# dan11003/tbv_slam_public

Measured on AMD Instinct MI355X. Metric: radar scan registrations/sec (400x3360 polar), higher is better.
Workload: dtype u8 filter / f32 search / f64 solve

## Files before the change

### tbv_slam_public_amd/csrc/kstrong.hip

```cpp
#include <cmath>

#include "polar_common.hpp"

namespace {

struct KStrongArgs {
  const uint8_t* polar;
  int rows, cols, stride, batch;
  long long batch_stride;
  int k, u_zmin, want_peaks, batch0;
  int32_t* sel_range;
  uint8_t* sel_intensity;
  int32_t* sel_count;
  uint8_t* is_peak;
  int32_t* row_valid;
  int min_range_bin;
  int dense_halo;
  uint32_t* row_keys;
  const long long* image_offsets;
};

__device__ __forceinline__ uint32_t swar_ge(uint32_t x, uint32_t tl4, bool thi) {
  const uint32_t g = ((x & 0x7f7f7f7fu) | 0x80808080u) - tl4;
  const uint32_t xh = x & 0x80808080u;
// ... 78 lines not shown
  const bool do_peaks = !STAGED && a.want_peaks && a.is_peak;
  uint8_t halo = 0;
  int halo_pos = 0;
  if (do_peaks && (lane < 6 || (lane >= 8 && lane < 14))) {
    const long long total = (long long)a.rows * a.stride;
    long long lin;
    if (lane < 6) {
      halo_pos = -6 + lane;
      lin = row_lin - 6 + lane;
      if (a.dense_halo) lin = r > 0 ? row_lin - a.stride + a.cols - 6 + lane : -1;
    } else {
      halo_pos = a.cols + (lane - 8);
      lin = row_lin + halo_pos;
      if (a.dense_halo) lin = r + 1 < a.rows ? row_lin + a.stride + (lane - 8) : total;
    }
    if (lin >= 0 && lin < total) halo = img[lin];
  }
  const int cols16 = (a.cols + 15) & ~15;
  uint32_t w[NCHUNK * 4];
  if (STAGED) {
#pragma unroll
    for (int c = 0; c < NCHUNK; c++) {
      uint4 v = make_uint4(0, 0, 0, 0);
      if ((c * 64 + lane) * 16 < cols16) v = *(const uint4*)(rowbuf + (c * 64 + lane) * 16);
      w[c * 4] = v.x; w[c * 4 + 1] = v.y; w[c * 4 + 2] = v.z; w[c * 4 + 3] = v.w;
    }
  } else {
    load_row<NCHUNK, VEC>(rowp, a.cols, lane, w, cfear_piece_inside_image(r, a.cols & ~15, a.rows, a.stride));
#pragma unroll
    for (int c = 0; c < NCHUNK; c++)
      *(uint4*)(rowbuf + (c * 64 + lane) * 16) = make_uint4(w[c * 4], w[c * 4 + 1], w[c * 4 + 2], w[c * 4 + 3]);
  }

  auto reload_row = [&](uint32_t (&x)[NCHUNK * 4]) {
#pragma unroll
    for (int c = 0; c < NCHUNK; c++) {
      uint4 v = make_uint4(0, 0, 0, 0);
      if (!STAGED || (c * 64 + lane) * 16 < cols16) v = *(const uint4*)(rowbuf + (c * 64 + lane) * 16);
      x[c * 4] = v.x; x[c * 4 + 1] = v.y; x[c * 4 + 2] = v.z; x[c * 4 + 3] = v.w;
    }
  };
  uint32_t bm[NCHUNK];
  {
    const uint32_t tz4 = (uint32_t)(a.u_zmin & 0x7f) * 0x01010101u;
    if (a.u_zmin & 0x80) candidate_bitmaps<NCHUNK, MASK, true>(w, tz4, a.cols, lane, bm);
    else candidate_bitmaps<NCHUNK, MASK, false>(w, tz4, a.cols, lane, bm);
  }
  int c_lane = 0;
#pragma unroll
  for (int c = 0; c < NCHUNK; c++) c_lane += __popc(bm[c]);
  const int c_incl = wave_incl_scan_i32(c_lane);
  const int n_ge = __builtin_amdgcn_readlane(c_incl, 63);
  int n_sel;
  int n_all;
  __builtin_amdgcn_fence(__ATOMIC_RELEASE, "wavefront");
  __builtin_amdgcn_wave_barrier();
  __builtin_amdgcn_fence(__ATOMIC_ACQUIRE, "wavefront");

  uint8_t* marker = (uint8_t*)hist;
  uint32_t* sexcl = hist + 64;
  uint32_t* spw = hist + 128;
  auto scatter_prepare = [&](const uint32_t (&bmx)[NCHUNK], int cnt_lane, int cnt_incl) {
    uint32_t pw[NP];
#pragma unroll
    for (int p = 0; p < NP; p++) pw[p] = (bmx[2 * p] >> 4) | (2 * p + 1 < NCHUNK ? bmx[2 * p + 1] : 0u);
    const int excl = cnt_incl - cnt_lane;
    ((uint32_t*)marker)[lane] = 0;
// ... 47 lines not shown
    const int s_incl = wave_incl_scan_i32(s_lane);
    const unsigned long long reach = __ballot(s_incl >= k);
    const int lc = __ffsll((long long)reach) - 1;
    int Tl = 0, gl = 0, el = 0;
    {
      int cum = s_incl - s_lane;
      const int hv[4] = {(int)h.w, (int)h.z, (int)h.y, (int)h.x};
      bool found = false;
#pragma unroll
      for (int j = 0; j < 4; j++) {
        if (!found && cum + hv[j] >= k) { Tl = 4 * (63 - lane) + 3 - j; gl = cum; el = hv[j]; found = true; }
        cum += hv[j];
      }
    }
    T = __builtin_amdgcn_readlane(Tl, lc);
    n_gt = __builtin_amdgcn_readlane(gl, lc);
    n_eq = __builtin_amdgcn_readlane(el, lc);
  };

  if (__builtin_expect(n_ge <= k || n_ge <= 64, 1)) {
    n_sel = min(n_ge, k);
    n_all = n_ge;
    if (__builtin_expect(n_ge <= 64, 1)) {
      scatter_to_lanes(bm, c_lane, c_incl, n_ge);
    } else {
      int slot = c_incl - c_lane;
      for_each_candidate<NCHUNK>(bm, lane, [&](int pos) { list[slot++] = ((uint32_t)rowbuf[pos] << 24) | (uint32_t)pos; });
    }
  } else {
    n_sel = k;
    n_all = k;
    int T = 0, n_gt = 0, n_eq = 0;
    bool have_list = false;
    uint32_t bt[NCHUNK];
    int t_lane = c_lane, t_incl = c_incl, n_c = n_ge;
#pragma unroll
    for (int c = 0; c < NCHUNK; c++) bt[c] = bm[c];
    bool exact = false;
    if (n_ge > 256) {
      int lo = a.u_zmin, c_lo = n_ge, hi = 256, c_hi = 0;
      bool first = true;
      while (hi - lo > 1) {
        int mid = first ? 256 - max(1, ((256 - lo) * 128) / c_lo) : (lo + hi) >> 1;
        mid = min(max(mid, lo + 1), hi - 1);
        first = false;
        const uint32_t tm4 = (uint32_t)(mid & 0x7f) * 0x01010101u;
        uint32_t bx[NCHUNK];
        {
          uint32_t wx[NCHUNK * 4];
          reload_row(wx);
          if (mid & 0x80) candidate_bitmaps<NCHUNK, MASK, true>(wx, tm4, a.cols, lane, bx);
          else candidate_bitmaps<NCHUNK, MASK, false>(wx, tm4, a.cols, lane, bx);
        }
        int x_lane = 0;
#pragma unroll
        for (int c = 0; c < NCHUNK; c++) x_lane += __popc(bx[c]);
        const int x_incl = wave_incl_scan_i32(x_lane);
        const int cnt = __builtin_amdgcn_readlane(x_incl, 63);
        if (cnt < k) { hi = mid; c_hi = cnt; }
        else if (cnt > 256) { lo = mid; c_lo = cnt; }
        else {
#pragma unroll
          for (int c = 0; c < NCHUNK; c++) bt[c] = bx[c];
          t_lane = x_lane; t_incl = x_incl; n_c = cnt;
          break;
        }
      }
      if (n_c > 256) { exact = true; T = lo; n_gt = c_hi; n_eq = c_lo - c_hi; }
    }
    if (!exact) {
      scatter_prepare(bt, t_lane, t_incl);
      scatter_carry = 0;
      uint32_t kr[4];
      bool kv[4];
      const int rounds = (n_c + 63) >> 6;
#pragma unroll
      for (int rd = 0; rd < 4; rd++) { kr[rd] = 0; kv[rd] = false; if (rd < rounds) kr[rd] = scatter_round(rd, n_c, kv[rd]); }
      __builtin_amdgcn_fence(__ATOMIC_ACQ_REL, "wavefront");
      __builtin_amdgcn_wave_barrier();
      *(uint4*)(hist + lane * 4) = make_uint4(0, 0, 0, 0);
      __builtin_amdgcn_fence(__ATOMIC_RELEASE, "wavefront");
      __builtin_amdgcn_wave_barrier();
#pragma unroll
      for (int rd = 0; rd < 4; rd++) if (kv[rd]) atomicAdd(&hist[kr[rd] >> 24], 1u);
      __builtin_amdgcn_fence(__ATOMIC_ACQ_REL, "wavefront");
      __builtin_amdgcn_wave_barrier();
      cut_from_hist(T, n_gt, n_eq);
      if (n_gt + n_eq <= 64) {
        int base = 0;
#pragma unroll
        for (int rd = 0; rd < 4; rd++) {
          const bool sel = kv[rd] && (int)(kr[rd] >> 24) >= T;
          const unsigned long long bal = __ballot(sel);
          if (sel) list[base + __popcll(bal & ((1ull << lane) - 1ull))] = kr[rd];
          base += __popcll(bal);
        }
        n_all = n_gt + n_eq;
        have_list = true;
      }
    }
    if (!have_list) {
    uint32_t wt[NCHUNK * 4];
    reload_row(wt);
    const int skip_eq = n_eq - (k - n_gt);
    const int thr_gt = T + 1;
    const uint32_t tg4 = (uint32_t)(thr_gt & 0x7f) * 0x01010101u;
    const bool tghi = (thr_gt & 0x80) != 0;
    const uint32_t te4 = (uint32_t)(T & 0x7f) * 0x01010101u;
    const bool tehi = (T & 0x80) != 0;
    int g_base = 0, e_base = 0;
#pragma unroll
    for (int c = 0; c < NCHUNK; c++) {
      uint32_t mg[4], me[4];
      int cg = 0, ce = 0;
#pragma unroll
      for (int d = 0; d < 4; d++) {
        const int i = c * 4 + d;
        const uint32_t valid = MASK ? ((bm[c] << (3 - d)) & 0x80808080u) : 0x80808080u;
        mg[d] = thr_gt > 255 ? 0u : (swar_ge(wt[i], tg4, tghi) & valid);
        me[d] = swar_ge(wt[i], te4, tehi) & valid & ~mg[d];
        cg += __popc(mg[d]);
        ce += __popc(me[d]);
      }
      const int packed = (ce << 16) | cg;
      const int incl = wave_incl_scan_i32(packed);
      const int tot = __builtin_amdgcn_readlane(incl, 63);
      const int excl = incl - packed;
      int g_run = g_base + (excl & 0xFFFF);
      int e_run = e_base + (excl >> 16);
      if (cg + ce) {
#pragma unroll
        for (int d = 0; d < 4; d++) {
          uint32_t mm = mg[d] | me[d];
          while (mm) {
            const int bit = __ffs(mm) - 1;
            mm &= mm - 1;
            const int by = bit >> 3;
            const bool is_eq = (me[d] >> bit) & 1u;
            const bool selected = !is_eq || e_run >= skip_eq;
            const int e_sel_before = e_run > skip_eq ? e_run - skip_eq : 0;
            if (selected) {
              const int pos = (c * 64 + lane) * 16 + d * 4 + by;
              list[g_run + e_sel_before] = (((wt[c * 4 + d] >> (8 * by)) & 0xffu) << 24) | (uint32_t)pos;
            }
            if (is_eq) e_run++; else g_run++;
          }
        }
      }
      g_base += tot & 0xFFFF;
      e_base += tot >> 16;
    }
    }
  }
  const int nq = (n_all + 3) & ~3;
  for (int j = n_all + lane; j < nq; j += 64) list[j] = 0xFFFFFFFFu;
  if (a.row_keys && lane < 2) hist[2 + lane] = 0;
  __builtin_amdgcn_fence(__ATOMIC_RELEASE, "wavefront");
  __builtin_amdgcn_wave_barrier();
  __builtin_amdgcn_fence(__ATOMIC_ACQUIRE, "wavefront");
  const int drop = n_all - n_sel;

  auto note_kept = [&](int m) {
    if (m >= 3 && m < a.cols - 3) {
      if (m < 16) atomicOr(&hist[0], 1u << m);
      if (m >= a.cols - 16) atomicOr(&hist[1], 1u << (m - (a.cols - 16)));
    }
  };
  if (__builtin_expect(do_peaks, 0)) {
    if (halo_pos != 0) rowbuf[halo_pos] = halo;
    if (lane < 2) hist[lane] = 0;
    __builtin_amdgcn_fence(__ATOMIC_RELEASE, "wavefront");
    __builtin_amdgcn_wave_barrier();
    if (drop == 0) {
      for (int j = lane; j < n_all; j += 64) note_kept((int)(list[j] & 0xFFFFFFu));
      __builtin_amdgcn_fence(__ATOMIC_ACQ_REL, "wavefront");
      __builtin_amdgcn_wave_barrier();
// ... 58 lines not shown
        a.is_peak[obase + rank] = pk ? 1 : 0;
        beyond_pk = beyond && pk;
      }
    }
    if (__builtin_expect(a.row_keys != nullptr, 1)) {
      if (beyond) atomicOr(&hist[2 + (rank >> 5)], 1u << (rank & 31));
      __builtin_amdgcn_fence(__ATOMIC_ACQ_REL, "wavefront");
      __builtin_amdgcn_wave_barrier();
      if (beyond) {
        const uint32_t m0 = hist[2], m1 = hist[3];
        const int idx = rank < 32 ? __popc(m0 & ((1u << rank) - 1u)) : __popc(m0) + __popc(m1 & ((1u << (rank - 32)) - 1u));
        a.row_keys[obase + idx] = key;
      }
    }
    nvalid += __popcll(__ballot(beyond));
    nvalid_pk += __popcll(__ballot(beyond_pk));
  }
  for (int j = n_sel + lane; j < k; j += 64) {
    if (a.sel_range) a.sel_range[obase + j] = -1;
    if (a.sel_intensity) a.sel_intensity[obase + j] = 0;
    if (do_peaks) a.is_peak[obase + j] = 0;
  }
  if (lane == 0) {
    if (a.row_valid) {
      a.row_valid[((long long)b * a.rows + r) * 2] = nvalid;
      a.row_valid[((long long)b * a.rows + r) * 2 + 1] = nvalid_pk;
    }
    if (a.sel_count) a.sel_count[(long long)b * a.rows + r] = n_sel;
  }
}

__host__ __device__ constexpr int kstrong_scratch_bytes(int nchunk) { return ((nchunk + 1) / 2 + 2) * 256 > 1024 ? ((nchunk + 1) / 2 + 2) * 256 : 1024; }

template <int NCHUNK, bool VEC, bool MASK>
__global__ __launch_bounds__(256, 7) void kstrongest_rows_kernel(const KStrongArgs a) {
  extern __shared__ __attribute__((aligned(16))) uint8_t smem[];
  const int wave = __builtin_amdgcn_readfirstlane(threadIdx.x >> 6), lane = threadIdx.x & 63;
  const int r = blockIdx.x * kRowsPerBlock + wave;
  if (r >= a.rows) return;
  const int b = a.batch0 + blockIdx.y;
  const uint8_t* img = a.polar + (a.image_offsets ? a.image_offsets[b] : (long long)b * a.batch_stride);
  const int kpad = max((a.k + 3) & ~3, 64);
  constexpr int kScratch = kstrong_scratch_bytes(NCHUNK);
  const int per_wave = NCHUNK * 1024 + 32 + kScratch + kpad * 4;
  uint8_t* rowbuf = smem + wave * per_wave + 16;
  uint32_t* hist = (uint32_t*)(smem + wave * per_wave + NCHUNK * 1024 + 32);
  uint32_t* list = (uint32_t*)(smem + wave * per_wave + NCHUNK * 1024 + 32 + kScratch);
  kstrong_row<NCHUNK, VEC, MASK, false>(a, r, b, img, rowbuf, hist, list, lane);
}

constexpr int kColsTile = 16;
constexpr int kColsWaves = 8;
constexpr int kCandCap = 256;
constexpr int kExtractPieces = 8;

template <typename Emit>
__device__ __forceinline__ void extract_candidates(const KStrongArgs& a, const uint32_t (&w)[kExtractPieces][4], const uint32_t p0,
                                                   const uint32_t step, const uint32_t n_pieces, const uint32_t seg_magic,
                                                   const int segs, Emit&& emit) {
  const uint32_t tz4 = (uint32_t)(a.u_zmin & 0x7f) * 0x01010101u;
  const bool thi = (a.u_zmin & 0x80) != 0;
  uint32_t cm[kExtractPieces / 2];
#pragma unroll
  for (int h = 0; h < kExtractPieces / 2; h++) cm[h] = 0;
#pragma unroll
  for (int u = 0; u < kExtractPieces; u++) {
    const uint32_t lo = __builtin_amdgcn_udot4(swar_ge(w[u][1], tz4, thi), 0x80402010u,
                                               __builtin_amdgcn_udot4(swar_ge(w[u][0], tz4, thi), 0x08040201u, 0u, false), false);
    const uint32_t hi = __builtin_amdgcn_udot4(swar_ge(w[u][3], tz4, thi), 0x80402010u,
// ... 710 lines not shown
```

### tbv_slam_public_amd/csrc/odometry.hip

```cpp
#include <algorithm>
#include <chrono>
#include <cmath>
#include <cstdlib>

#include "covfit.hpp"
#include "registration.hpp"

extern "C" int cfear_keyframe_based_fuse(const double diff_xyt[3], int32_t use_keyframe, double min_keyframe_dist,
                                         double min_keyframe_rot_deg) {
  if (!use_keyframe) return 1;
  const double tn = std::sqrt(diff_xyt[0] * diff_xyt[0] + diff_xyt[1] * diff_xyt[1]);
  const double rot = std::fabs(diff_xyt[2]);
  return (tn > min_keyframe_dist || rot > (min_keyframe_rot_deg * M_PI / 180.0)) ? 1 : 0;
}
extern "C" int cfear_acc_vel_sanity_check(const double tmot_prev_xy[2], const double tmot_curr_xy[2]) {
  return pose2d_acc_vel_sane(tmot_prev_xy, tmot_curr_xy);
}

namespace {

struct Keyframe { int slab; Aff2 pose; uint64_t idx = 0; };
struct StreamState {
  Aff2 T_prev = aff_identity(), Tmot = aff_identity(), Tcurrent = aff_identity();
  std::vector<Keyframe> keyframes;
// ... 24 lines not shown
  size_t slab_bytes = 0;
  DevBuf<uint8_t> d_polar;
  DevBuf<uint8_t> d_rot;
  bool fused_decode = false;
  DevBuf<uint32_t> d_decode_stats;
  PinnedBuf<uint32_t> h_decode_stats;
  bool decode_measured[2] = {false, false};
  int decode_hold = 0;
  DevBuf<char> d_sel;
  DevBuf<float> d_xyzi2[2];
  DevBuf<int32_t> d_npts2[2];
  float* d_xyzi = nullptr;
  int32_t* d_npts = nullptr;
  bool fused = false;
  bool fused_cfar = false;
  int row_k = 0;
  DevBuf<uint32_t> d_rowpts2[2];
  DevBuf<int32_t> d_rowcnt2[2];
  DevBuf<int64_t> d_offsets2[2];
  PinnedBuf<int64_t> h_offsets;
  std::vector<int64_t> prefetched_offsets;
  DevBuf<float> d_pk2[2];
  DevBuf<int32_t> d_npk2[2];
  float* d_pk = nullptr;
  int32_t* d_npk = nullptr;
  DevBuf<double> d_mot;
  PinnedBuf<double> h_mot;
  PinnedBuf<int32_t> h_npk;
  std::vector<int> last_slab;
  int cur_buf = 0;
  const uint8_t* prefetched = nullptr;
  Event ev_results;
  Event ev_jobs;
  DevBuf<char> d_slabs, d_surf_jobs, d_reg_jobs;
  DevBuf<char> d_out;
  PinnedBuf<char> h_out;
  size_t out_bytes = 0;
  int32_t* d_npts_out = nullptr;
  cfear_reg_result* d_results = nullptr;
  int32_t* d_status = nullptr;
  int32_t* d_ncells = nullptr;
  DevBuf<char> d_surf_scratch, d_reg_scratch;
  PinnedBuf<char> h_surf_jobs, h_reg_jobs;
  cfear_reg_result* h_results = nullptr;
  int32_t* h_status = nullptr;
  int32_t* h_npts = nullptr;
  int32_t* h_ncells = nullptr;
  DevBuf<cfear_reg_result> d_samples;
  PinnedBuf<cfear_reg_result> h_samples;
  CovFit fit;
  std::vector<double> cov;
  std::vector<int32_t> cov_sampled;
  std::vector<StreamState> streams;
  int big_regs = 0;
  std::vector<double> cost_est, cost_tmp;
  std::vector<int> job_slot;
  std::vector<ScanView> views;
};

extern "C" int cfear_odometry_destroy(cfear_odometry* od) {
  if (!od) return CFEAR_OK;
  (void)hipSetDevice(od->ctx->device);
  (void)hipStreamSynchronize(od->ctx->stream);
  delete od;
  return CFEAR_OK;
}

extern "C" int cfear_odometry_create(cfear_ctx* ctx, int32_t n_streams, const cfear_polar_desc* desc,
                                     const cfear_odometry_params* par, cfear_odometry** out) {
  if (!ctx) return CFEAR_ERR_INVALID_ARGUMENT;
  if (!desc || !par || !out || n_streams < 1) return cfear_set_error(ctx, CFEAR_ERR_INVALID_ARGUMENT, "null argument");
  *out = nullptr;
  if (desc->batch != n_streams) return cfear_set_error(ctx, CFEAR_ERR_INVALID_ARGUMENT, "desc.batch must equal n_streams");
  if (par->submap_scan_size < 1 || par->submap_scan_size + 1 > kRegMaxScans)
    return cfear_set_error(ctx, CFEAR_ERR_INVALID_ARGUMENT, "submap_scan_size must be in [1,%d]", kRegMaxScans - 1);
  if (!(par->res > 0.05f)) return cfear_set_error(ctx, CFEAR_ERR_INVALID_ARGUMENT, "res must be > 0.05");
  if (par->estimate_cov_by_sampling && (par->cov_sampling.samples_per_axis < 1 || par->cov_sampling.samples_per_axis > 15))
    return cfear_set_error(ctx, CFEAR_ERR_INVALID_ARGUMENT, "cov_sampling.samples_per_axis must be in [1,15]");
  {
    const int fcols = par->rotate_ccw ? desc->rows : desc->cols;
    if (desc->rows <= 0 || desc->cols <= 0 || desc->stride < desc->cols ||
        (n_streams > 1 && desc->batch_stride < (int64_t)desc->rows * desc->stride))
      return cfear_set_error(ctx, CFEAR_ERR_INVALID_ARGUMENT, "bad polar descriptor");
    if (fcols > 8192) return cfear_set_error(ctx, CFEAR_ERR_INVALID_ARGUMENT, "more than 8192 range bins unsupported");
    if (par->filter_type == CFEAR_FILTER_CACFAR) {
      if (par->cacfar.window_size < 1 || par->cacfar.nb_guard_cells < 0 || !(par->cacfar.range_res > 0.f))
        return cfear_set_error(ctx, CFEAR_ERR_INVALID_ARGUMENT, "bad CFAR parameters");
    } else if (par->filter_type == CFEAR_FILTER_KSTRONG) {
      if (par->kstrong.k_strongest < 1 || par->kstrong.k_strongest > 1024)
        return cfear_set_error(ctx, CFEAR_ERR_INVALID_ARGUMENT, "k_strongest must be in [1,1024]");
      if (!(par->kstrong.range_res > 0.f) || !(par->kstrong.min_distance >= 0.f))
        return cfear_set_error(ctx, CFEAR_ERR_INVALID_ARGUMENT, "range_res must be > 0 and min_distance >= 0");
    } else {
      return cfear_set_error(ctx, CFEAR_ERR_INVALID_ARGUMENT, "unknown filter_type %d", par->filter_type);
    }
  }
// ... 26 lines not shown
  od->fused_cfar = par->filter_type == CFEAR_FILTER_CACFAR && !par->keep_nodes && rows <= 4096;
  if (od->fused_cfar) {
    od->row_k = std::min((od->desc.cols + 3) / 4 * 4, 1024);
    for (int i = 0; i < 2; i++) {
      dev(od->d_rowpts2[i], (size_t)B * rows * od->row_k * 4);
      dev(od->d_rowcnt2[i], (size_t)B * rows * 8);
    }
  }
  if (od->fused) {
    for (int i = 0; i < 2; i++) {
      dev(od->d_rowpts2[i], nsel * 4);
      dev(od->d_rowcnt2[i], (size_t)B * rows * 8);
      dev(od->d_offsets2[i], (size_t)B * 8);
    }
    pin(od->h_offsets, (size_t)B * 8 * 2);
  } else {
    dev(od->d_sel, nsel * 4 + 2 * (nsel + 256) + (size_t)B * rows * 4 + 1024);
  }
  if (par->keep_nodes) {
    for (int i = 0; i < 2; i++) {
      dev(od->d_pk2[i], (size_t)B * od->cap_points * 16);
      dev(od->d_npk2[i], (size_t)B * 4);
    }
    dev(od->d_mot, (size_t)B * 3 * sizeof(double));
    pin(od->h_mot, (size_t)B * 3 * sizeof(double));
    pin(od->h_npk, (size_t)B * 4);
  }
  od->last_slab.assign(B, -1);
  for (int i = 0; i < 2; i++) {
    dev(od->d_xyzi2[i], (size_t)B * od->cap_points * 16);
    dev(od->d_npts2[i], (size_t)B * 4);
  }
  ok = ok && (od->ev_results = make_event(hipEventDisableTiming)) && (od->ev_jobs = make_event(hipEventDisableTiming)) &&
       (od->copy_stream = make_stream_nonblocking());
  dev(od->d_slabs, (size_t)B * od->slabs_per_stream * od->slab_bytes);
  dev(od->d_surf_jobs, (size_t)B * cfear_surface_job_bytes());
  const size_t reg_job_room = std::max(sizeof(RegJob), reg_job_stride(par->submap_scan_size + 1));
  dev(od->d_reg_jobs, (size_t)B * reg_job_room);
  od->out_bytes = (size_t)B * (sizeof(cfear_reg_result) + 12);
  dev(od->d_out, od->out_bytes);
  pin(od->h_out, od->out_bytes);
  if (ok) {
    auto carve = [&](char* base) {
      struct P { cfear_reg_result* r; int32_t *st, *nc, *np; } q;
      q.r = (cfear_reg_result*)base;
      q.st = (int32_t*)(base + (size_t)B * sizeof(cfear_reg_result));
      q.nc = q.st + B; q.np = q.nc + B;
      return q;
    };
    const auto d = carve(od->d_out.get()), h = carve(od->h_out.get());
    od->d_results = d.r; od->d_status = d.st; od->d_ncells = d.nc; od->d_npts_out = d.np;
    od->h_results = h.r; od->h_status = h.st; od->h_ncells = h.nc; od->h_npts = h.np;
  }
  dev(od->d_surf_scratch, (size_t)B * cfear_surface_scratch_bytes(od->cap_points));
  dev(od->d_reg_scratch, (size_t)B * reg_scratch_bytes(par->submap_scan_size * od->cell_cap));
  pin(od->h_surf_jobs, (size_t)B * cfear_surface_job_bytes());
  pin(od->h_reg_jobs, (size_t)B * reg_job_room);
  if (par->estimate_cov_by_sampling) {
    od->fit.prepare(par->cov_sampling.samples_per_axis, par->cov_sampling.xy_range * 0.5, par->cov_sampling.yaw_range * 0.5);
    dev(od->d_samples, (size_t)B * od->fit.m * sizeof(cfear_reg_result));
    pin(od->h_samples, (size_t)B * od->fit.m * sizeof(cfear_reg_result));
  }
  od->cov.assign((size_t)B * 36, 0.0);
  for (int b = 0; b < B; b++)
    for (int k = 0; k < 6; k++) od->cov[(size_t)b * 36 + k * 7] = 1.0;
  od->cov_sampled.assign(B, 0);
  if (!ok) return cfear_set_error(ctx, CFEAR_ERR_HIP, "odometry buffers: allocation failed");
  od->streams.resize(B);
  od->cost_est.assign(B, 0.0);
  od->views.resize((size_t)B * od->slabs_per_stream);
  for (int b = 0; b < B; b++) {
    for (int s = 0; s < od->slabs_per_stream; s++) {
      od->views[(size_t)b * od->slabs_per_stream + s] =
          cfear_scan_view(od->d_slabs.get() + ((size_t)b * od->slabs_per_stream + s) * od->slab_bytes, od->cell_cap);
      od->streams[b].free_slabs.push_back(od->slabs_per_stream - 1 - s);
    }
  }
  *out = od.release();
  return CFEAR_OK;
}

static int run_filter(cfear_odometry* od, const uint8_t* polar, int buf, const int64_t* offsets = nullptr) {
  cfear_ctx* ctx = od->ctx;
  const int B = od->n_streams, rows = od->desc.rows, k = od->par.kstrong.k_strongest;
  const cfear_odometry_params& par = od->par;
  const uint8_t* d_polar = polar;
  cfear_polar_desc dd = od->in_desc;
  const int64_t* d_offsets = nullptr;
  if (offsets) {
    if (!od->fused || par.rotate_ccw || !cfear_is_device_ptr(polar))
      return cfear_set_error(ctx, CFEAR_ERR_INVALID_ARGUMENT, "image offsets need device images, the k-strongest filter "
                             "(k <= 64, no keep_nodes) and rows = azimuths");
    int64_t* h = od->h_offsets.get() + (size_t)buf * B;
    memcpy(h, offsets, (size_t)B * 8);
    CFEAR_HIP_CHECK(ctx, hipMemcpyAsync(od->d_offsets2[buf].get(), h, (size_t)B * 8, hipMemcpyHostToDevice, ctx->stream));
    d_offsets = od->d_offsets2[buf].get();
  }
  if (!cfear_is_device_ptr(polar)) {
    const size_t img_bytes = (size_t)od->in_desc.rows * od->in_desc.stride;
    if (!od->d_polar && !(od->d_polar = dev_alloc<uint8_t>(img_bytes * B))) return cfear_set_error(ctx, CFEAR_ERR_HIP, "staging allocation failed");
    const int64_t bs = B > 1 ? od->in_desc.batch_stride : (int64_t)img_bytes;
    if (bs == (int64_t)img_bytes) {
      CFEAR_HIP_CHECK(ctx, hipMemcpyAsync(od->d_polar.get(), polar, img_bytes * B, hipMemcpyHostToDevice, ctx->stream));
    } else {
      for (int b = 0; b < B; b++)
        CFEAR_HIP_CHECK(ctx, hipMemcpyAsync(od->d_polar.get() + (size_t)b * img_bytes, polar + (size_t)b * bs, img_bytes,
                                            hipMemcpyHostToDevice, ctx->stream));
    }
    d_polar = od->d_polar.get();
    dd.batch_stride = (int64_t)img_bytes;
  }
  od->decode_measured[buf] = false;
  if (od->fused_decode && od->decode_hold > 0) od->decode_hold--;
  else if (od->fused_decode && cfear_kstrong_cols_preferred(d_polar, &dd, &par.kstrong)) {
    cfear_kstrong_params kp = par.kstrong;
    kp.want_peaks = 0;
    cfear_kstrong_fused fz;
    fz.row_keys = od->d_rowpts2[buf].get();
    fz.row_valid = od->d_rowcnt2[buf].get();
    fz.cand_stats = od->d_decode_stats.get() + 64 * buf;
    const int rc = cfear_kstrong_cols_device(ctx, d_polar, &dd, &kp, &fz);
    if (rc != CFEAR_OK) return rc;
    CFEAR_HIP_CHECK(ctx, hipMemcpyAsync(od->h_decode_stats.get() + 64 * buf, fz.cand_stats, 64 * 4, hipMemcpyDeviceToHost, ctx->stream));
    od->decode_measured[buf] = true;
    return CFEAR_OK;
  }
  if (par.rotate_ccw && od->fused_cfar && ctx->opt[CFEAR_OPT_FUSED_DECODE] != 0 && B >= 16 &&
      cfear_cacfar_cols_supported(d_polar, &dd, &par.cacfar)) {
// ... 20 lines not shown
      return cfear_cacfar_device(ctx, d_polar, &dd, &cp, nullptr, nullptr, od->cap_points, nullptr, &fz);
    }
    return cfear_cacfar_device(ctx, d_polar, &dd, &cp, od->d_xyzi2[buf].get(), od->d_npts2[buf].get(), od->cap_points, nullptr);
  }
  const size_t nsel = (size_t)B * rows * k;
  cfear_kstrong_out o{};
  if (od->fused) {
    cfear_kstrong_params kp = par.kstrong;
    kp.want_peaks = 0;
    cfear_kstrong_fused fz;
    fz.row_keys = od->d_rowpts2[buf].get();
    fz.row_valid = od->d_rowcnt2[buf].get();
    fz.image_offsets = d_offsets;
    return cfear_kstrong_device(ctx, d_polar, &dd, &kp, &o, par.rotate_ccw != 0, &fz);
  }
  o.sel_range = (int32_t*)od->d_sel.get();
  o.sel_intensity = (uint8_t*)(od->d_sel.get() + nsel * 4);
  o.sel_count = (int32_t*)(od->d_sel.get() + nsel * 4 + (nsel + 255) / 256 * 256);
  o.xyzi = od->d_xyzi2[buf].get();
  o.n_points = od->d_npts2[buf].get();
  cfear_kstrong_params kp = par.kstrong;
  kp.want_peaks = 0;
  if (par.keep_nodes) {
    kp.want_peaks = 1;
    o.is_peak = (uint8_t*)(od->d_sel.get() + nsel * 4 + (nsel + 255) / 256 * 256 + (size_t)B * rows * 4 + 256);
    o.xyzi_peaks = od->d_pk2[buf].get();
    o.n_peaks = od->d_npk2[buf].get();
  }
  if (od->cap_points != rows * k)
    return cfear_set_error(ctx, CFEAR_ERR_CAPACITY, "rows*k = %d exceeds %d points per scan", rows * k, od->cap_points);
  return cfear_kstrong_device(ctx, d_polar, &dd, &kp, &o, par.rotate_ccw != 0);
}

extern "C" int cfear_odometry_get_covariance(cfear_odometry* od, double* cov, int32_t* sampled) {
  if (!od || !cov) return CFEAR_ERR_INVALID_ARGUMENT;
  memcpy(cov, od->cov.data(), od->cov.size() * sizeof(double));
  if (sampled) memcpy(sampled, od->cov_sampled.data(), od->cov_sampled.size() * sizeof(int32_t));
  return CFEAR_OK;
}

extern "C" int cfear_odometry_process(cfear_odometry* od, const uint8_t* polar, cfear_frame_info* info) {
  return cfear_odometry_process_prefetch(od, polar, nullptr, info);
}

static int process_frame(cfear_odometry* od, const uint8_t* polar, const uint8_t* polar_next, const cfear_sc_cloud* clouds,
                         const cfear_sc_cloud* peaks, cfear_frame_info* info, const int64_t* offsets = nullptr,
                         const int64_t* offsets_next = nullptr);

extern "C" int cfear_odometry_process_offsets(cfear_odometry* od, const uint8_t* base, const int64_t* offsets,
                                              const int64_t* offsets_next, cfear_frame_info* info) {
  if (!od || !base || !offsets || !info) return CFEAR_ERR_INVALID_ARGUMENT;
  return process_frame(od, base, offsets_next ? base : nullptr, nullptr, nullptr, info, offsets, offsets_next);
}

extern "C" int cfear_odometry_discard_prefetch(cfear_odometry* od) {
  if (!od) return CFEAR_ERR_INVALID_ARGUMENT;
  od->prefetched = nullptr;
  od->prefetched_offsets.clear();
  return CFEAR_OK;
}

extern "C" int cfear_odometry_process_prefetch(cfear_odometry* od, const uint8_t* polar, const uint8_t* polar_next,
                                               cfear_frame_info* info) {
  if (!od || !polar || !info) return CFEAR_ERR_INVALID_ARGUMENT;
  return process_frame(od, polar, polar_next, nullptr, nullptr, info);
}

extern "C" int cfear_odometry_process_clouds(cfear_odometry* od, const cfear_sc_cloud* clouds, const cfear_sc_cloud* peaks,
                                             cfear_frame_info* info) {
  if (!od || !clouds || !info) return CFEAR_ERR_INVALID_ARGUMENT;
  return process_frame(od, nullptr, nullptr, clouds, peaks, info);
}

static int load_clouds(cfear_odometry* od, const cfear_sc_cloud* clouds, float* d_dst, int32_t* d_n, int32_t* h_tmp) {
  cfear_ctx* ctx = od->ctx;
  const int B = od->n_streams;
  for (int b = 0; b < B; b++) {
    const int n = clouds ? clouds[b].n : 0;
    if (n < 0 || (n > 0 && !clouds[b].xyzi)) return cfear_set_error(ctx, CFEAR_ERR_INVALID_ARGUMENT, "stream %d: null cloud", b);
    if (n > od->cap_points) return cfear_set_error(ctx, CFEAR_ERR_CAPACITY, "stream %d: %d points > %d", b, n, od->cap_points);
    h_tmp[b] = n;
    if (n > 0) {
      const bool dev = cfear_is_device_ptr(clouds[b].xyzi);
      CFEAR_HIP_CHECK(ctx, hipMemcpyAsync(d_dst + (size_t)b * od->cap_points * 4, clouds[b].xyzi, (size_t)n * 16,
                                          dev ? hipMemcpyDeviceToDevice : hipMemcpyHostToDevice, ctx->stream));
    }
  }
  CFEAR_HIP_CHECK(ctx, hipMemcpyAsync(d_n, h_tmp, (size_t)B * 4, hipMemcpyHostToDevice, ctx->stream));
  CFEAR_HIP_CHECK(ctx, hipStreamSynchronize(ctx->stream));
  return CFEAR_OK;
}
// ... 34 lines not shown
  cfear_ctx* ctx = od->ctx;
  g_tl.on = ctx->opt[CFEAR_OPT_HOST_TIMELINE] != 0;
  g_tl.start();
  CFEAR_HIP_CHECK(ctx, hipSetDevice(ctx->device));
  const int B = od->n_streams;
  const cfear_odometry_params& par = od->par;
  int rc;
  if (clouds) {
    od->prefetched = nullptr;
    rc = load_clouds(od, clouds, od->d_xyzi2[od->cur_buf].get(), od->d_npts2[od->cur_buf].get(), od->h_npts);
    if (rc != CFEAR_OK) return rc;
    if (par.keep_nodes) {
      rc = load_clouds(od, peaks, od->d_pk2[od->cur_buf].get(), od->d_npk2[od->cur_buf].get(), od->h_npk.get());
      if (rc != CFEAR_OK) return rc;
    }
  } else if (od->prefetched == polar &&
             (offsets ? (od->prefetched_offsets.size() == (size_t)B &&
                         memcmp(od->prefetched_offsets.data(), offsets, (size_t)B * 8) == 0)
                      : od->prefetched_offsets.empty())) {
    od->cur_buf ^= 1;
  } else {
    rc = run_filter(od, polar, od->cur_buf, offsets);
    if (rc != CFEAR_OK) return rc;
  }
  od->prefetched = nullptr;
  od->prefetched_offsets.clear();
  od->d_xyzi = od->d_xyzi2[od->cur_buf].get();
  od->d_npts = od->d_npts2[od->cur_buf].get();
  od->d_pk = od->d_pk2[od->cur_buf].get();
  od->d_npk = od->d_npk2[od->cur_buf].get();
  const bool rows_mode = (od->fused || od->fused_cfar) && !clouds;
  const size_t sjb = cfear_surface_job_bytes();
  for (int b = 0; b < B; b++)
    if (od->streams[b].free_slabs.empty()) return cfear_set_error(ctx, CFEAR_ERR_CAPACITY, "stream %d: no free scan slab", b);
  for (int b = 0; b < B; b++) {
    StreamState& st = od->streams[b];
    st.cur_slab = st.free_slabs.back();
    st.free_slabs.pop_back();
    double mot[3];
    aff_to_xyt(st.Tmot, mot);
    od->last_slab[b] = st.cur_slab;
    if (par.keep_nodes) { od->h_mot[3 * b] = mot[0]; od->h_mot[3 * b + 1] = mot[1]; od->h_mot[3 * b + 2] = mot[2]; }
    if (rows_mode)
      cfear_surface_fill_job_rows(od->h_surf_jobs.get() + (size_t)b * sjb, od->d_xyzi + (size_t)b * od->cap_points * 4, od->d_npts_out + b,
                                  od->d_rowpts2[od->cur_buf].get() + (size_t)b * od->desc.rows * od->row_k,
                                  od->d_rowcnt2[od->cur_buf].get() + (size_t)b * od->desc.rows * 2, od->desc.rows,
                                  od->row_k, par.compensate, mot,
                                  od->views[(size_t)b * od->slabs_per_stream + st.cur_slab]);
    else
      cfear_surface_fill_job(od->h_surf_jobs.get() + (size_t)b * sjb, od->d_xyzi + (size_t)b * od->cap_points * 4,
                             od->d_npts + b, 0, par.compensate, mot, od->views[(size_t)b * od->slabs_per_stream + st.cur_slab]);
  }
  auto fail = [&](int code) {
    for (int b = 0; b < B; b++) {
      StreamState& st = od->streams[b];
      if (st.cur_slab >= 0) { st.free_slabs.push_back(st.cur_slab); st.cur_slab = -1; }
    }
    return code;
  };
#define OD_CHECK(expr)                                                                                        \
  do {                                                                                                        \
    hipError_t _e = (expr);                                                                                   \
    if (_e != hipSuccess)                                                                                     \
      return fail(cfear_set_error(ctx, CFEAR_ERR_HIP, "%s failed: %s (%s:%d)", #expr, hipGetErrorString(_e), __FILE__, __LINE__)); \
  } while (0)
  OD_CHECK(hipMemcpyAsync(od->d_surf_jobs.get(), od->h_surf_jobs.get(), (size_t)B * sjb, hipMemcpyHostToDevice, ctx->stream));
  cfear_feature_params fp{};
  fp.radius = par.res;
  fp.downsample_factor = par.downsample_factor;
  fp.origin[0] = fp.origin[1] = 0.0;
  fp.weight_intensity = par.weight_intensity;
  fp.ccw = par.radar_ccw;
  cfear_surface_polar sp;
  if (rows_mode) {
    double *d_cos = nullptr, *d_sin = nullptr;
    rc = cfear_trig_tables(ctx, od->desc.rows, &d_cos, &d_sin);
    if (rc != CFEAR_OK) return fail(rc);
    sp.cos_t = d_cos; sp.sin_t = d_sin;
    sp.rows = od->desc.rows; sp.k = od->row_k;
    if (od->fused_cfar) {
      sp.range_res = (double)par.cacfar.range_res; sp.range_off = 0.0;
    } else {
      sp.range_res = (double)par.kstrong.range_res; sp.range_off = sp.range_res / 2.0;
    }
  }
  rc = cfear_surface_launch(ctx, od->d_surf_jobs.get(), B, &fp, od->d_surf_scratch.get(), od->d_status, od->d_ncells, od->cell_cap, od->cap_points, rows_mode ? &sp : nullptr);
  if (rc != CFEAR_OK) return fail(rc);
  g_tl.mark(0);
  const size_t rjb = reg_job_stride(par.submap_scan_size + 1);
  int n_jobs = 0;
  std::vector<ScanView> views(kRegMaxScans);
  std::vector<double> poses(3 * (size_t)kRegMaxScans);
  std::vector<double>& est = od->cost_est;
  double cut[4] = {0.0, 0.0, 0.0, 0.0};
  {
    std::vector<double>& tmp = od->cost_tmp;
    tmp.assign(est.begin(), est.end());
    if (B >= 8) {
      const size_t ks[4] = {(size_t)B * 97 / 100, (size_t)B * 3 / 4, (size_t)B / 2, (size_t)B / 4};
// ... 22 lines not shown
    StreamState& st = od->streams[b];
    const int ns = (int)st.keyframes.size() + 1;
    for (int i = 0; i < ns - 1; i++) {
      views[i] = od->views[(size_t)b * od->slabs_per_stream + st.keyframes[i].slab];
      aff_to_xyt(st.keyframes[i].pose, &poses[3 * i]);
    }
    views[ns - 1] = od->views[(size_t)b * od->slabs_per_stream + st.cur_slab];
    aff_to_xyt(st.Tguess, &poses[3 * (ns - 1)]);
    st.job = cls_off[slot[b] & 7] + (slot[b] >> 3);
    cfear_reg_fill_job(od->h_reg_jobs.get() + (size_t)st.job * rjb, views.data(), ns, poses.data());
  }
  if (n_jobs > 0) {
    OD_CHECK(hipMemcpyAsync(od->d_reg_jobs.get(), od->h_reg_jobs.get(), (size_t)n_jobs * rjb, hipMemcpyHostToDevice, od->copy_stream.get()));
    OD_CHECK(hipEventRecord(od->ev_jobs.get(), od->copy_stream.get()));
  }
  g_tl.mark(1);
  auto launch_register = [&](bool big_pass) -> int {
    RegLaunchHint hint;
    hint.big_pass = big_pass;
    int lrc = cfear_register_launch(ctx, od->d_reg_jobs.get(), n_jobs, &par.reg, par.submap_scan_size * od->cell_cap,
                                    od->d_reg_scratch.get(), od->d_results, nullptr, rjb, hint);
    if (lrc != CFEAR_OK) return lrc;
    if (par.estimate_cov_by_sampling) {
      RegCostMode mode;
      mode.samples_per_axis = od->fit.n;
      mode.n_samples = od->fit.m;
      mode.xy_half = par.cov_sampling.xy_range * 0.5;
      mode.yaw_half = par.cov_sampling.yaw_range * 0.5;
      mode.blocks_per_job = 1;
      mode.prior = od->d_results;
      lrc = cfear_register_launch(ctx, od->d_reg_jobs.get(), n_jobs, &par.reg, par.submap_scan_size * od->cell_cap,
                                  od->d_reg_scratch.get(), od->d_samples.get(), &mode, rjb, hint);
      if (lrc != CFEAR_OK) return lrc;
      if (hipMemcpyAsync(od->h_samples.get(), od->d_samples.get(), (size_t)n_jobs * od->fit.m * sizeof(cfear_reg_result),
                         hipMemcpyDeviceToHost, ctx->stream) != hipSuccess)
        return cfear_set_error(ctx, CFEAR_ERR_HIP, "sample read-back failed");
    }
    return CFEAR_OK;
  };
  const bool launched_big = od->big_regs > 0;
  if (n_jobs > 0) {
    OD_CHECK(hipStreamWaitEvent(ctx->stream, od->ev_jobs.get(), 0));
    rc = launch_register(launched_big);
    if (rc != CFEAR_OK) return fail(rc);
  }
  if (par.keep_nodes) {
    if (par.compensate) {
      OD_CHECK(hipMemcpyAsync(od->d_mot.get(), od->h_mot.get(), (size_t)B * 3 * sizeof(double), hipMemcpyHostToDevice, ctx->stream));
      rc = cfear_compensate_batch_device(ctx, od->d_pk, (size_t)od->cap_points, od->d_npk, od->d_mot.get(), B, od->cap_points, par.radar_ccw);
      if (rc != CFEAR_OK) return fail(rc);
    }
    OD_CHECK(hipMemcpyAsync(od->h_npk.get(), od->d_npk, (size_t)B * 4, hipMemcpyDeviceToHost, ctx->stream));
  }
  if (!rows_mode)
    OD_CHECK(hipMemcpyAsync(od->d_npts_out, od->d_npts, (size_t)B * 4, hipMemcpyDeviceToDevice, ctx->stream));
  OD_CHECK(hipMemcpyAsync(od->h_out.get(), od->d_out.get(), od->out_bytes, hipMemcpyDeviceToHost, ctx->stream));
  OD_CHECK(hipEventRecord(od->ev_results.get(), ctx->stream));
  int prefetch_rc = CFEAR_OK;
  if (polar_next) {
    prefetch_rc = run_filter(od, polar_next, od->cur_buf ^ 1, offsets_next);
    if (prefetch_rc == CFEAR_OK) {
      od->prefetched = polar_next;
      if (offsets_next) od->prefetched_offsets.assign(offsets_next, offsets_next + B);
    }
  }
  g_tl.mark(2);
  OD_CHECK(hipEventSynchronize(od->ev_results.get()));
  g_tl.mark(3);
  if (n_jobs > 0 && !launched_big) {
    bool retry = false;
    for (int j = 0; j < n_jobs && !retry; j++) retry = od->h_results[j].status == CFEAR_ERR_CAPACITY && od->h_results[j].reserved != 0.0;
    if (retry) {
      rc = launch_register(true);
      if (rc != CFEAR_OK) return fail(rc);
      OD_CHECK(hipMemcpyAsync(od->h_results, od->d_results, (size_t)n_jobs * sizeof(cfear_reg_result), hipMemcpyDeviceToHost, ctx->stream));
      OD_CHECK(hipStreamSynchronize(ctx->stream));
    }
  }
  if (od->decode_measured[od->cur_buf]) {
    od->decode_measured[od->cur_buf] = false;
    uint64_t cands = 0;
    for (int k = 0; k < 64; k++) cands += od->h_decode_stats[64 * od->cur_buf + k];
    if ((double)cands > kDecodeDense * (double)B * (double)od->desc.rows) od->decode_hold = kDecodeHold;
  }
  int first_error = CFEAR_OK;
  bool saw_big = false;
  for (int b = 0; b < B; b++) {
    StreamState& st = od->streams[b];
    cfear_frame_info& fi = info[b];
    memset(&fi, 0, sizeof(fi));
    fi.n_points = od->h_npts[b];
    fi.n_cells = od->h_ncells[b];
    st.has_constraint = false;
    if (od->h_status[b] != CFEAR_OK) {
      if (first_error == CFEAR_OK)
        first_error = cfear_set_error(ctx, od->h_status[b], "stream %d: surface points failed (%s)", b, cfear_status_string(od->h_status[b]));
      fi.reg_status = od->h_status[b];
      st.free_slabs.push_back(st.cur_slab);
      aff_to_xyt(st.Tcurrent, fi.pose);
      continue;
    }
    if (st.job < 0) {
      st.keyframes.push_back(Keyframe{st.cur_slab, aff_identity(), st.n_keyframes++});
      fi.keyframe_added = 1;
      fi.reg_status = 1;
      aff_to_xyt(st.Tcurrent, fi.pose);
// ... 163 lines not shown
```

### tbv_slam_public_amd/csrc/surface.hip

```cpp
#include <cfloat>
#include <cmath>
#include <memory>
#include <type_traits>

#include "common.hpp"
#include "fastmath.hpp"
#include "gridsort.hpp"

namespace {

constexpr int kSurfThreads = kGridSortThreads;
constexpr int kMaxPoints = kGridSortMaxPoints;
constexpr int kMaxGridRows = 4096;
constexpr int kPerThread = kMaxPoints / kSurfThreads;
constexpr size_t kLdsRowbegOff = (size_t)kMaxPoints * 8 + 16;
constexpr size_t kLdsSmallOff = (kLdsRowbegOff + (size_t)(kMaxGridRows + 1) * 4 + 15) / 16 * 16;
constexpr size_t kLdsTotal = kLdsSmallOff + 256 + 64 + 32;

struct SurfJob {
  float4* xyzi;
  const int32_t* n_ptr;
  int32_t n_host;
  int32_t compensate;
  double mot[3];
// ... 1262 lines not shown
        }
      }
    };
    tier(std::integral_constant<int, 16>{}, 0, n16);
    STAMP(14);
    tier(std::integral_constant<int, 4>{}, n16, n4);
    STAMP(15);
    tier(std::integral_constant<int, 1>{}, n4, nlist);
    __syncthreads();
    ya = yb;
  }
  return true;
  };
  if (!(wbyte ? cells_phase(std::true_type{}) : cells_phase(std::false_type{}))) return;
  STAMP(8);
  if (tid == 0) {
    scr.hdr->route = kRouteFast;
    scr.hdr->n = n; scr.hdr->V = V; scr.hdr->dbx = dbx; scr.hdr->dby = dby;
    scr.hdr->path = path | (n_slabs > 1 ? CFEAR_SURF_PATH_SLABS : 0u) | ((uint32_t)min(n_slabs, 255) << CFEAR_SURF_PATH_SLAB_COUNT_SHIFT);
  }
}

__global__ __launch_bounds__(kFastThreads, 4) void surface_sort_kernel(const SurfJob* __restrict__ jobs, const SurfCommon cm) {
  surface_sort_job<32>(jobs, cm);
}
__global__ __launch_bounds__(kFastThreads, 4) void surface_sort_mixed_kernel(const SurfJob* __restrict__ jobs, const SurfCommon cm) {
  const SurfScratch scr = scratch_of(cm.scratch + (size_t)blockIdx.x * cm.scratch_stride, cm.scratch_cap);
  if (scr.hdr->n > 32 * kFastThreads) surface_sort_job<64>(jobs, cm);
  else surface_sort_job<32>(jobs, cm);
}

constexpr int kFinishThreads = 256;

__global__ __launch_bounds__(kFinishThreads) void surface_finish_kernel(const SurfJob* __restrict__ jobs, const SurfCommon cm) {
  extern __shared__ __attribute__((aligned(16))) uint8_t smem[];
  __shared__ int red_i2[2][kFinishThreads / 64];
  const int tid = threadIdx.x, wave = tid >> 6, lane = tid & 63;
  const int job_id = blockIdx.x;
  const SurfScratch scr = scratch_of(cm.scratch + (size_t)job_id * cm.scratch_stride, cm.scratch_cap);
  if (job_id == 0 && tid == 0) cm.fallback[0] = 0;
  if (scr.hdr->route != kRouteFast) return;
  const SurfJob job = jobs[job_id];
  const int V = scr.hdr->V;
  int run = 0;
  int cnt_next = tid < V ? gload<int32_t>(scr.coff + tid) : 0;
  for (int v0 = 0, rnd = 0; v0 < V; v0 += kFinishThreads, rnd ^= 1) {
    const int v = v0 + tid;
    const int cnt = cnt_next;
    cnt_next = v + kFinishThreads < V ? gload<int32_t>(scr.coff + v + kFinishThreads) : 0;
    TmpCell t;
    int f = 0;
    if (v < V && cnt >= 6) {
      const char* src = (const char*)&scr.tmp[v];
      const g_f64x2 a = gload<g_f64x2>(src), b = gload<g_f64x2>(src + 16), c = gload<g_f64x2>(src + 32);
      const g_f32x2 d = gload<g_f32x2>(src + 48);
      const Moments mo{cnt, a.x, a.y, b.x, b.y, c.x, c.y};
      f = finish_cell(mo, (double)d.x, (double)d.y, cm.origin[0], cm.origin[1], t);
    }
    const int inc = wave_incl_scan_i32(f);
    if (lane == 63) red_i2[rnd][wave] = inc;
    __syncthreads();
    int off = run + inc - f;
    for (int wv = 0; wv < kFinishThreads / 64; wv++) { if (wv < wave) off += red_i2[rnd][wv]; run += red_i2[rnd][wv]; }
    if (f && off < job.out.cap) {
      gstore<g_f32x2>(job.out.mean_f + off, g_f32x2{(float)t.mean[0], (float)t.mean[1]});
      gstore<g_f64x2>(job.out.mean + off, g_f64x2{t.mean[0], t.mean[1]});
      gstore<g_f64x2>(job.out.normal + off, g_f64x2{t.normal[0], t.normal[1]});
// ... 517 lines not shown
```

Before: 1.391 million.

## Move H2D/D2H transfers to copy stream, trim kstrong registers, tune finish occupancy

Host-to-device copies for offsets and surface jobs now go on the separate copy stream and are joined to the main stream with events. Result read-back is issued on the copy stream after the next frame's filter prefetch has been enqueued, so the copy can overlap compute. The k-strongest kernel now reloads one chunk at a time from LDS instead of holding a full row copy, and runs scatter_prepare directly instead of copying bitmaps, which cuts register pressure. It also adds an optional padding macro and sets a minimum-occupancy launch bound on surface_finish_kernel. The extra events and syncs add stream-ordering complexity, and the error paths now drain both streams.

```diff
diff --git a/tbv_slam_public_amd/csrc/kstrong.hip b/tbv_slam_public_amd/csrc/kstrong.hip
--- a/tbv_slam_public_amd/csrc/kstrong.hip
+++ b/tbv_slam_public_amd/csrc/kstrong.hip
@@ -134,7 +134,14 @@
       *(uint4*)(rowbuf + (c * 64 + lane) * 16) = make_uint4(w[c * 4], w[c * 4 + 1], w[c * 4 + 2], w[c * 4 + 3]);
   }
 
+  auto reload_chunk = [&](const int c, uint32_t (&x)[4]) {
+    asm volatile("" ::: "memory");
+    uint4 v = make_uint4(0, 0, 0, 0);
+    if (!STAGED || (c * 64 + lane) * 16 < cols16) v = *(const uint4*)(rowbuf + (c * 64 + lane) * 16);
+    x[0] = v.x; x[1] = v.y; x[2] = v.z; x[3] = v.w;
+  };
   auto reload_row = [&](uint32_t (&x)[NCHUNK * 4]) {
+    asm volatile("" ::: "memory");
 #pragma unroll
     for (int c = 0; c < NCHUNK; c++) {
       uint4 v = make_uint4(0, 0, 0, 0);
@@ -248,11 +255,8 @@
     n_all = k;
     int T = 0, n_gt = 0, n_eq = 0;
     bool have_list = false;
-    uint32_t bt[NCHUNK];
-    int t_lane = c_lane, t_incl = c_incl, n_c = n_ge;
-#pragma unroll
-    for (int c = 0; c < NCHUNK; c++) bt[c] = bm[c];
-    bool exact = false;
+    int n_c = n_ge;
+    bool exact = false, prepared = false;
     if (n_ge > 256) {
       int lo = a.u_zmin, c_lo = n_ge, hi = 256, c_hi = 0;
       bool first = true;
@@ -265,8 +269,12 @@
         {
           uint32_t wx[NCHUNK * 4];
           reload_row(wx);
-          if (mid & 0x80) candidate_bitmaps<NCHUNK, MASK, true>(wx, tm4, a.cols, lane, bx);
-          else candidate_bitmaps<NCHUNK, MASK, false>(wx, tm4, a.cols, lane, bx);
+          if (mid & 0x80) candidate_bitmaps<NCHUNK, false, true>(wx, tm4, a.cols, lane, bx);
+          else candidate_bitmaps<NCHUNK, false, false>(wx, tm4, a.cols, lane, bx);
+          if (MASK) {
+#pragma unroll
+            for (int c = 0; c < NCHUNK; c++) bx[c] &= bm[c];
+          }
         }
         int x_lane = 0;
 #pragma unroll
@@ -276,16 +284,15 @@
         if (cnt < k) { hi = mid; c_hi = cnt; }
         else if (cnt > 256) { lo = mid; c_lo = cnt; }
         else {
-#pragma unroll
-          for (int c = 0; c < NCHUNK; c++) bt[c] = bx[c];
-          t_lane = x_lane; t_incl = x_incl; n_c = cnt;
+          scatter_prepare(bx, x_lane, x_incl);
+          n_c = cnt; prepared = true;
           break;
         }
       }
       if (n_c > 256) { exact = true; T = lo; n_gt = c_hi; n_eq = c_lo - c_hi; }
     }
     if (!exact) {
-      scatter_prepare(bt, t_lane, t_incl);
+      if (!prepared) scatter_prepare(bm, c_lane, c_incl);
       scatter_carry = 0;
       uint32_t kr[4];
       bool kv[4];
@@ -316,8 +323,6 @@
       }
     }
     if (!have_list) {
-    uint32_t wt[NCHUNK * 4];
-    reload_row(wt);
     const int skip_eq = n_eq - (k - n_gt);
     const int thr_gt = T + 1;
     const uint32_t tg4 = (uint32_t)(thr_gt & 0x7f) * 0x01010101u;
@@ -327,14 +332,15 @@
     int g_base = 0, e_base = 0;
 #pragma unroll
     for (int c = 0; c < NCHUNK; c++) {
+      uint32_t wt[4];
+      reload_chunk(c, wt);
       uint32_t mg[4], me[4];
       int cg = 0, ce = 0;
 #pragma unroll
       for (int d = 0; d < 4; d++) {
-        const int i = c * 4 + d;
         const uint32_t valid = MASK ? ((bm[c] << (3 - d)) & 0x80808080u) : 0x80808080u;
-        mg[d] = thr_gt > 255 ? 0u : (swar_ge(wt[i], tg4, tghi) & valid);
-        me[d] = swar_ge(wt[i], te4, tehi) & valid & ~mg[d];
+        mg[d] = thr_gt > 255 ? 0u : (swar_ge(wt[d], tg4, tghi) & valid);
+        me[d] = swar_ge(wt[d], te4, tehi) & valid & ~mg[d];
         cg += __popc(mg[d]);
         ce += __popc(me[d]);
       }
@@ -357,7 +363,7 @@
             const int e_sel_before = e_run > skip_eq ? e_run - skip_eq : 0;
             if (selected) {
               const int pos = (c * 64 + lane) * 16 + d * 4 + by;
-              list[g_run + e_sel_before] = (((wt[c * 4 + d] >> (8 * by)) & 0xffu) << 24) | (uint32_t)pos;
+              list[g_run + e_sel_before] = (((wt[d] >> (8 * by)) & 0xffu) << 24) | (uint32_t)pos;
             }
             if (is_eq) e_run++; else g_run++;
           }
@@ -482,9 +488,16 @@
 
 __host__ __device__ constexpr int kstrong_scratch_bytes(int nchunk) { return ((nchunk + 1) / 2 + 2) * 256 > 1024 ? ((nchunk + 1) / 2 + 2) * 256 : 1024; }
 
+#ifndef CFEAR_KSTRONG_HEAD_PAD
+#define CFEAR_KSTRONG_HEAD_PAD 0
+#endif
+
 template <int NCHUNK, bool VEC, bool MASK>
 __global__ __launch_bounds__(256, 7) void kstrongest_rows_kernel(const KStrongArgs a) {
   extern __shared__ __attribute__((aligned(16))) uint8_t smem[];
+#if CFEAR_KSTRONG_HEAD_PAD > 0
+  asm volatile(".rept %0\n\ts_nop 0\n\t.endr" ::"n"(CFEAR_KSTRONG_HEAD_PAD / 4));
+#endif
   const int wave = __builtin_amdgcn_readfirstlane(threadIdx.x >> 6), lane = threadIdx.x & 63;
   const int r = blockIdx.x * kRowsPerBlock + wave;
   if (r >= a.rows) return;
diff --git a/tbv_slam_public_amd/csrc/odometry.hip b/tbv_slam_public_amd/csrc/odometry.hip
--- a/tbv_slam_public_amd/csrc/odometry.hip
+++ b/tbv_slam_public_amd/csrc/odometry.hip
@@ -80,6 +80,10 @@
   const uint8_t* prefetched = nullptr;
   Event ev_results;
   Event ev_jobs;
+  Event ev_surf_jobs;
+  Event ev_offsets[2];
+  Event ev_frame;
+  bool readback_on_copy_stream = false;
   DevBuf<char> d_slabs, d_surf_jobs, d_reg_jobs;
   DevBuf<char> d_out;
   PinnedBuf<char> h_out;
@@ -106,10 +110,15 @@
   std::vector<ScanView> views;
 };
 
+static void drain_streams(cfear_odometry* od) {
+  if (od->copy_stream) (void)hipStreamSynchronize(od->copy_stream.get());
+  (void)hipStreamSynchronize(od->ctx->stream);
+}
+
 extern "C" int cfear_odometry_destroy(cfear_odometry* od) {
   if (!od) return CFEAR_OK;
   (void)hipSetDevice(od->ctx->device);
-  (void)hipStreamSynchronize(od->ctx->stream);
+  drain_streams(od);
   delete od;
   return CFEAR_OK;
 }
@@ -202,7 +211,10 @@
     dev(od->d_npts2[i], (size_t)B * 4);
   }
   ok = ok && (od->ev_results = make_event(hipEventDisableTiming)) && (od->ev_jobs = make_event(hipEventDisableTiming)) &&
+       (od->ev_surf_jobs = make_event(hipEventDisableTiming)) && (od->ev_offsets[0] = make_event(hipEventDisableTiming)) &&
+       (od->ev_offsets[1] = make_event(hipEventDisableTiming)) && (od->ev_frame = make_event(hipEventDisableTiming)) &&
        (od->copy_stream = make_stream_nonblocking());
+  od->readback_on_copy_stream = ctx->stream != nullptr && ctx->stream != hipStreamLegacy && ctx->stream != hipStreamPerThread;
   dev(od->d_slabs, (size_t)B * od->slabs_per_stream * od->slab_bytes);
   dev(od->d_surf_jobs, (size_t)B * cfear_surface_job_bytes());
   const size_t reg_job_room = std::max(sizeof(RegJob), reg_job_stride(par->submap_scan_size + 1));
@@ -250,7 +262,7 @@
   return CFEAR_OK;
 }
 
-static int run_filter(cfear_odometry* od, const uint8_t* polar, int buf, const int64_t* offsets = nullptr) {
+static int run_filter_enqueue(cfear_odometry* od, const uint8_t* polar, int buf, const int64_t* offsets) {
   cfear_ctx* ctx = od->ctx;
   const int B = od->n_streams, rows = od->desc.rows, k = od->par.kstrong.k_strongest;
   const cfear_odometry_params& par = od->par;
@@ -263,7 +275,9 @@
                              "(k <= 64, no keep_nodes) and rows = azimuths");
     int64_t* h = od->h_offsets.get() + (size_t)buf * B;
     memcpy(h, offsets, (size_t)B * 8);
-    CFEAR_HIP_CHECK(ctx, hipMemcpyAsync(od->d_offsets2[buf].get(), h, (size_t)B * 8, hipMemcpyHostToDevice, ctx->stream));
+    CFEAR_HIP_CHECK(ctx, hipMemcpyAsync(od->d_offsets2[buf].get(), h, (size_t)B * 8, hipMemcpyHostToDevice, od->copy_stream.get()));
+    CFEAR_HIP_CHECK(ctx, hipEventRecord(od->ev_offsets[buf].get(), od->copy_stream.get()));
+    CFEAR_HIP_CHECK(ctx, hipStreamWaitEvent(ctx->stream, od->ev_offsets[buf].get(), 0));
     d_offsets = od->d_offsets2[buf].get();
   }
   if (!cfear_is_device_ptr(polar)) {
@@ -350,6 +364,12 @@
   return cfear_kstrong_device(ctx, d_polar, &dd, &kp, &o, par.rotate_ccw != 0);
 }
 
+static int run_filter(cfear_odometry* od, const uint8_t* polar, int buf, const int64_t* offsets = nullptr) {
+  const int rc = run_filter_enqueue(od, polar, buf, offsets);
+  if (rc != CFEAR_OK && offsets) drain_streams(od);
+  return rc;
+}
+
 extern "C" int cfear_odometry_get_covariance(cfear_odometry* od, double* cov, int32_t* sampled) {
   if (!od || !cov) return CFEAR_ERR_INVALID_ARGUMENT;
   memcpy(cov, od->cov.data(), od->cov.size() * sizeof(double));
@@ -375,6 +395,8 @@
   if (!od) return CFEAR_ERR_INVALID_ARGUMENT;
   od->prefetched = nullptr;
   od->prefetched_offsets.clear();
+  (void)hipSetDevice(od->ctx->device);
+  drain_streams(od);
   return CFEAR_OK;
 }
 
@@ -475,7 +497,10 @@
   const bool rows_mode = (od->fused || od->fused_cfar) && !clouds;
   const size_t sjb = cfear_surface_job_bytes();
   for (int b = 0; b < B; b++)
-    if (od->streams[b].free_slabs.empty()) return cfear_set_error(ctx, CFEAR_ERR_CAPACITY, "stream %d: no free scan slab", b);
+    if (od->streams[b].free_slabs.empty()) {
+      drain_streams(od);
+      return cfear_set_error(ctx, CFEAR_ERR_CAPACITY, "stream %d: no free scan slab", b);
+    }
   for (int b = 0; b < B; b++) {
     StreamState& st = od->streams[b];
     st.cur_slab = st.free_slabs.back();
@@ -495,6 +520,7 @@
                              od->d_npts + b, 0, par.compensate, mot, od->views[(size_t)b * od->slabs_per_stream + st.cur_slab]);
   }
   auto fail = [&](int code) {
+    drain_streams(od);
     for (int b = 0; b < B; b++) {
       StreamState& st = od->streams[b];
       if (st.cur_slab >= 0) { st.free_slabs.push_back(st.cur_slab); st.cur_slab = -1; }
@@ -507,7 +533,9 @@
     if (_e != hipSuccess)                                                                                     \
       return fail(cfear_set_error(ctx, CFEAR_ERR_HIP, "%s failed: %s (%s:%d)", #expr, hipGetErrorString(_e), __FILE__, __LINE__)); \
   } while (0)
-  OD_CHECK(hipMemcpyAsync(od->d_surf_jobs.get(), od->h_surf_jobs.get(), (size_t)B * sjb, hipMemcpyHostToDevice, ctx->stream));
+  OD_CHECK(hipMemcpyAsync(od->d_surf_jobs.get(), od->h_surf_jobs.get(), (size_t)B * sjb, hipMemcpyHostToDevice, od->copy_stream.get()));
+  OD_CHECK(hipEventRecord(od->ev_surf_jobs.get(), od->copy_stream.get()));
+  OD_CHECK(hipStreamWaitEvent(ctx->stream, od->ev_surf_jobs.get(), 0));
   cfear_feature_params fp{};
   fp.radius = par.res;
   fp.downsample_factor = par.downsample_factor;
@@ -596,10 +624,14 @@
       lrc = cfear_register_launch(ctx, od->d_reg_jobs.get(), n_jobs, &par.reg, par.submap_scan_size * od->cell_cap,
                                   od->d_reg_scratch.get(), od->d_samples.get(), &mode, rjb, hint);
       if (lrc != CFEAR_OK) return lrc;
-      if (hipMemcpyAsync(od->h_samples.get(), od->d_samples.get(), (size_t)n_jobs * od->fit.m * sizeof(cfear_reg_result),
-                         hipMemcpyDeviceToHost, ctx->stream) != hipSuccess)
-        return cfear_set_error(ctx, CFEAR_ERR_HIP, "sample read-back failed");
-    }
+    }
+    return CFEAR_OK;
+  };
+  auto read_samples = [&](hipStream_t s) -> int {
+    if (!par.estimate_cov_by_sampling || n_jobs == 0) return CFEAR_OK;
+    if (hipMemcpyAsync(od->h_samples.get(), od->d_samples.get(), (size_t)n_jobs * od->fit.m * sizeof(cfear_reg_result),
+                       hipMemcpyDeviceToHost, s) != hipSuccess)
+      return cfear_set_error(ctx, CFEAR_ERR_HIP, "sample read-back failed");
     return CFEAR_OK;
   };
   const bool launched_big = od->big_regs > 0;
@@ -614,12 +646,24 @@
       rc = cfear_compensate_batch_device(ctx, od->d_pk, (size_t)od->cap_points, od->d_npk, od->d_mot.get(), B, od->cap_points, par.radar_ccw);
       if (rc != CFEAR_OK) return fail(rc);
     }
-    OD_CHECK(hipMemcpyAsync(od->h_npk.get(), od->d_npk, (size_t)B * 4, hipMemcpyDeviceToHost, ctx->stream));
   }
   if (!rows_mode)
     OD_CHECK(hipMemcpyAsync(od->d_npts_out, od->d_npts, (size_t)B * 4, hipMemcpyDeviceToDevice, ctx->stream));
-  OD_CHECK(hipMemcpyAsync(od->h_out.get(), od->d_out.get(), od->out_bytes, hipMemcpyDeviceToHost, ctx->stream));
-  OD_CHECK(hipEventRecord(od->ev_results.get(), ctx->stream));
+  auto read_back = [&](hipStream_t s) -> int {
+    const int src = read_samples(s);
+    if (src != CFEAR_OK) return src;
+    hipError_t e = hipSuccess;
+    if (par.keep_nodes) e = hipMemcpyAsync(od->h_npk.get(), od->d_npk, (size_t)B * 4, hipMemcpyDeviceToHost, s);
+    if (e == hipSuccess) e = hipMemcpyAsync(od->h_out.get(), od->d_out.get(), od->out_bytes, hipMemcpyDeviceToHost, s);
+    if (e == hipSuccess) e = hipEventRecord(od->ev_results.get(), s);
+    return e == hipSuccess ? CFEAR_OK : cfear_set_error(ctx, CFEAR_ERR_HIP, "result read-back failed: %s", hipGetErrorString(e));
+  };
+  if (od->readback_on_copy_stream) {
+    OD_CHECK(hipEventRecord(od->ev_frame.get(), ctx->stream));
+  } else {
+    rc = read_back(ctx->stream);
+    if (rc != CFEAR_OK) return fail(rc);
+  }
   int prefetch_rc = CFEAR_OK;
   if (polar_next) {
     prefetch_rc = run_filter(od, polar_next, od->cur_buf ^ 1, offsets_next);
@@ -627,6 +671,11 @@
       od->prefetched = polar_next;
       if (offsets_next) od->prefetched_offsets.assign(offsets_next, offsets_next + B);
     }
+  }
+  if (od->readback_on_copy_stream) {
+    OD_CHECK(hipStreamWaitEvent(od->copy_stream.get(), od->ev_frame.get(), 0));
+    rc = read_back(od->copy_stream.get());
+    if (rc != CFEAR_OK) return fail(rc);
   }
   g_tl.mark(2);
   OD_CHECK(hipEventSynchronize(od->ev_results.get()));
@@ -636,6 +685,8 @@
     for (int j = 0; j < n_jobs && !retry; j++) retry = od->h_results[j].status == CFEAR_ERR_CAPACITY && od->h_results[j].reserved != 0.0;
     if (retry) {
       rc = launch_register(true);
+      if (rc != CFEAR_OK) return fail(rc);
+      rc = read_samples(ctx->stream);
       if (rc != CFEAR_OK) return fail(rc);
       OD_CHECK(hipMemcpyAsync(od->h_results, od->d_results, (size_t)n_jobs * sizeof(cfear_reg_result), hipMemcpyDeviceToHost, ctx->stream));
       OD_CHECK(hipStreamSynchronize(ctx->stream));
diff --git a/tbv_slam_public_amd/csrc/surface.hip b/tbv_slam_public_amd/csrc/surface.hip
--- a/tbv_slam_public_amd/csrc/surface.hip
+++ b/tbv_slam_public_amd/csrc/surface.hip
@@ -1318,7 +1318,7 @@
 
 constexpr int kFinishThreads = 256;
 
-__global__ __launch_bounds__(kFinishThreads) void surface_finish_kernel(const SurfJob* __restrict__ jobs, const SurfCommon cm) {
+__global__ __launch_bounds__(kFinishThreads, 5) void surface_finish_kernel(const SurfJob* __restrict__ jobs, const SurfCommon cm) {
   extern __shared__ __attribute__((aligned(16))) uint8_t smem[];
   __shared__ int red_i2[2][kFinishThreads / 64];
   const int tid = threadIdx.x, wave = tid >> 6, lane = tid & 63;
```

Measured after the change: 1.437 million (median of 6 runs). +3.3%, better.
